# colonelwatch/ESP32-fluid-simulation

Measured on AMD Instinct MI355X. Metric: cell-iters/sec (SOR sweep), higher is better.
Workload: dtype f32

## Files before the change

esp32-fluid-simulation_amd/__init__.py:

```python
from . import _capi as capi
from ._capi import LIB_PATH, SflError, build_library
from .solver import (BatchSolver, HostPath, Solver, comm_unique_id, device_count, device_info, plan_poisson,
                     member_params, member_stops, slab_rows, sor_pass_plan, stdout_to_stderr, FLOW_STATS_DTYPE,
                     FLOW_STATS_STRIP_COLS, FLOW_STATS_CHUNK_ROWS, FIELD_DISTANCE_DTYPE, DIST_THREADS, DIST_ITEM_LOADS,
                     DIST_VELOCITY_LANE_CELLS, DIST_PRESSURE_LANE_CELLS, DIST_DYE_LANE_CELLS, ENV_BLOCK_WORDS,
                     ENV_GROUP_MEMBERS, View, PALETTE_GREY, PALETTE_HEAT, PALETTE_BLUE_WHITE_RED)

__all__ = ["capi", "LIB_PATH", "SflError", "build_library", "BatchSolver", "HostPath", "Solver",
           "comm_unique_id", "device_count", "device_info", "member_params", "member_stops", "plan_poisson", "slab_rows",
           "sor_pass_plan", "stdout_to_stderr", "FLOW_STATS_DTYPE", "FLOW_STATS_STRIP_COLS", "FLOW_STATS_CHUNK_ROWS",
           "FIELD_DISTANCE_DTYPE", "DIST_THREADS", "DIST_ITEM_LOADS", "DIST_VELOCITY_LANE_CELLS", "DIST_PRESSURE_LANE_CELLS",
           "DIST_DYE_LANE_CELLS", "ENV_BLOCK_WORDS", "ENV_GROUP_MEMBERS", "View", "PALETTE_GREY", "PALETTE_HEAT",
           "PALETTE_BLUE_WHITE_RED"]
```

esp32-fluid-simulation_amd/_capi.py:

```python
from __future__ import annotations

import ctypes as C
import os
import subprocess

_PKG = os.path.dirname(os.path.abspath(__file__))
LIB_PATH = os.path.join(_PKG, "lib", "libsfl_hip.so")

OK, ERR_INVALID, ERR_HIP, ERR_RCCL, ERR_NOMEM, ERR_STATE, ERR_HALO = 0, -1, -2, -3, -4, -5, -6
FIELD_VELOCITY, FIELD_COLOR, FIELD_DIVERGENCE, FIELD_PRESSURE = 0, 1, 2, 3
OPT_SOR_KERNEL, OPT_SOR_FUSE, OPT_ADVECT_HALO, OPT_SOR_ROWS, OPT_TRANSPORT = 0, 1, 2, 3, 4
OPT_SOR_LANE_CELLS = 5
OPT_SOR_HALO = 6
OPT_FUSE_PROJECTION = 7
OPT_ADVECT_KERNEL = 9
OPT_FUSE_DIVERGENCE = 10
OPT_SMALL_GRID = 11
OPT_EMULATE_WIRE_US = 12
OPT_STEP_SEAMS = 14
OPT_LAST_EARLY_ROWS = 17
OPT_HALO_TIMEOUT_MS = 18
OPT_EXCHANGE_SCHEDULE = 19
SCHEDULE_AUTO, SCHEDULE_IN_LINE, SCHEDULE_BY_EVENT, SCHEDULE_IN_TIME = 0, 1, 2, 3
OPT_MEASURED_WIRE_US = 20
# ... 127 lines not shown
    "sfl_distance": (_i, [_ctx, _ctx, _i, C.POINTER(FieldDistance)]),
    "sfl_step": (_i, [_ctx, _f, _f, _i, _f]),
    "sfl_step_n": (_i, [_ctx, _i, _f, _f, _i, _f]),
    "sfl_queue_forces": (_i, [_ctx, _pi, _pf, _i]),
    "sfl_queue_drags": (_i, [_ctx, C.c_void_p, _i]),
    "sfl_queue_forces_at": (_i, [_ctx, _i, _pi, _pf, _i]),
    "sfl_queue_drags_at": (_i, [_ctx, _i, C.c_void_p, _i]),
    "sfl_forces_pending": (_i, [_ctx, _pi, _pi]),
    "sfl_forget_forces": (_i, [_ctx]),
    "sfl_setup_sketch_fields": (_i, [_ctx]),
    "sfl_render_rgb565": (_i, [_ctx, _i, _i, C.POINTER(C.c_uint16), _sz]),
    "sfl_synchronize": (_i, [_ctx]),
    "sfl_timer_start": (_i, [_ctx]),
    "sfl_timer_stop": (_i, [_ctx, _pf]),
    "sfl_last_solve_info": (_i, [_ctx, _pi, _pi, _pi]),
    "sfl_batch_create": (_i, [C.POINTER(_ctx), _i, _i, _i, _i]),
    "sfl_batch_create_large": (_i, [C.POINTER(_ctx), _i, _i, _i, _i]),
    "sfl_batch_is_large": (_i, [_ctx, _pi]),
    "sfl_batch_destroy": (_i, [_ctx]),
    "sfl_batch_shape": (_i, [_ctx, _pi, _pi, _pi]),
    "sfl_batch_upload": (_i, [_ctx, _i, _i, _i, C.c_void_p, _sz]),
    "sfl_batch_download": (_i, [_ctx, _i, _i, _i, C.c_void_p, _sz]),
    "sfl_batch_field_device_ptr": (_i, [_ctx, _i, C.POINTER(C.c_void_p)]),
    "sfl_batch_queue_forces": (_i, [_ctx, _pi, _pi, _pf, _i]),
    "sfl_batch_queue_forces_at": (_i, [_ctx, _i, _pi, _pi, _pf, _i]),
    "sfl_batch_forces_pending": (_i, [_ctx, _pi, _pi]),
    "sfl_batch_forget_forces": (_i, [_ctx]),
    "sfl_batch_step_n": (_i, [_ctx, _i, _f, _f, _i, _f]),
    "sfl_batch_poisson_solve": (_i, [_ctx, _f, _i, _f]),
    "sfl_batch_step_n_each": (_i, [_ctx, _i, C.POINTER(MemberParams)]),
# ... 54 lines not shown
```

esp32-fluid-simulation_amd/csrc/sor_executor.cpp:

```cpp
#include "transport.h"

namespace sfl {
namespace host {

static bool quarter_omega_is_exact(float omega) { return (-0.25f * omega) * -4.0f == omega; }

sfl::SorParams sor_params(const sfl_context *c, float dx, float omega)
{
    sfl::SorParams prm;
    prm.dx = dx;
    prm.omega = omega;
    prm.one_minus_omega = 1.0f - omega;
    prm.neg_quarter_omega = -0.25f * omega;
    prm.fold = c->opt.sor_fold && quarter_omega_is_exact(omega) ? 1 : 0;
    return prm;
}

int effective_fuse(const sfl_context *c)
{
    int f = c->opt.sor_fuse;
    if (f == 0) {
        const int64_t cells = (int64_t)min_owned_rows(c) * c->dim_x;
        f = cells >= 12000000 ? 16 : cells >= 3000000 ? 10 : 8;
    }
// ... 389 lines not shown
        const sfl_plan_step &last = progs[k].back();
        if (last.kind != SFL_STEP_SOR) tail = 0;
        if (c->rank > 0) tail = std::min(tail, c->g0 - last.g_begin);
        if (c->rank < c->nranks - 1) tail = std::min(tail, last.g_end - c->g1);
    }
    for (sfl_context *c : peers) c->p_ghost_valid = tail > 0 ? tail : 0;
    if (timed_solve >= 0) {
        SFL_TRY(use_device(ctx));
        HIP_TRY(hipEventRecord(tuner.ev[2 * timed_solve + 1], ctx->stream));
    }
    return SFL_OK;
}

}
}
```

esp32-fluid-simulation_amd/csrc/sor_fused.hip:

```cpp
#include <cstdio>
#include <cstdlib>

#include "kernels.h"
#include "sor_stream_core.h"

#ifndef SFL_DX_PART
#define SFL_DX_PART (-1)
#endif

namespace sfl {
namespace {

constexpr int kWavesPerBlock = 4;
#ifndef SFL_NT_STORE_CELLS
#define SFL_NT_STORE_CELLS (24u << 20)
#endif
constexpr size_t kNtStoreCells = SFL_NT_STORE_CELLS;
constexpr int kFlipTiles = 1;
constexpr int kThreads = 64 * kWavesPerBlock;

#include "sor_lane.h"

#ifndef SFL_MIN_WAVES_DEEP
#define SFL_MIN_WAVES_DEEP 3
#endif
// ... 11 lines not shown
        B bk;
        bk.rs_p = __builtin_amdgcn_make_buffer_rsrc(const_cast<float *>(ZERO_IN ? d : p_in), 0, records, 0x00020000);
        bk.rs_d = __builtin_amdgcn_make_buffer_rsrc(const_cast<float *>(d), 0, records, 0x00020000);
        bk.rs_out = __builtin_amdgcn_make_buffer_rsrc(p_out, 0, records, 0x00020000);
        bk.dim_x = g.dim_x;
        bk.gdim_y = g.gdim_y;
        bk.grow0 = g.grow0;
        bk.row_lo = max(g.grow0, 0);
        bk.row_hi = min(g.grow0 + g.lrows, g.gdim_y);
        bk.row_sign = 1;
        bk.prio_on = sender ? 2 : t.rotate;
        bk.start_turns();
        bk.setup(ring_base, lane, x0, t.halo_cols);
        return bk;
    };
    if (sor::tile_touches_boundary(t, rect, g.gdim_y)) {
        B bk = backend();
        sor::Consts<B> c{bk.splat(prm.dx), bk.splat(prm.omega), bk.splat(prm.one_minus_omega), bk.splat(prm.neg_quarter_omega)};
        const auto eca = bk.edge_cell(lane, x0, 0);
        const auto ecb = bk.edge_cell(lane, x0, 1);
        sor::stream_tile<B, NS, true, DX1, ZERO_IN>(bk, c, eca, ecb, r0, r1);
        return 1;
    }
    if (sor::tile_may_flip(t, rect)) {
        B bk = backend();
        bk.row_sign = -1;
        sor::Consts<B> c{bk.splat(prm.dx), bk.splat(prm.omega), bk.splat(prm.one_minus_omega), bk.splat(prm.neg_quarter_omega)};
        const sor::EdgeCell<B> none{};
        sor::stream_tile<B, NS, false, DX1, ZERO_IN, true>(bk, c, none, none, 1 - r1, 1 - r0);
        return 2;
    }
    B bk = backend();
    sor::Consts<B> c{bk.splat(prm.dx), bk.splat(prm.omega), bk.splat(prm.one_minus_omega), bk.splat(prm.neg_quarter_omega)};
    const sor::EdgeCell<B> none{};
    sor::stream_tile<B, NS, false, DX1, ZERO_IN>(bk, c, none, none, r0, r1);
    return 0;
}

__device__ __forceinline__ int tile_of_wave(int wave, int free_blocks)
{
    int block = blockIdx.x;
    if (block < free_blocks) {
        const int per = free_blocks >> 3, rem = free_blocks & 7;
        const int xcd = block & 7, idx = block >> 3;
        block = xcd * per + min(xcd, rem) + idx;
    }
    return block * kWavesPerBlock + wave;
}

template <class B, int NS, bool DX1, bool ZERO_IN>
__global__ void __launch_bounds__(kThreads) __attribute__((amdgpu_waves_per_eu(min_waves_per_simd(NS))))
// ... 65 lines not shown
inline int device_simds()
{
    static int cached = 0;
    if (cached) return cached;
    int dev = 0, cus = 0;
    if (hipGetDevice(&dev) != hipSuccess ||
        hipDeviceGetAttribute(&cus, hipDeviceAttributeMultiprocessorCount, dev) != hipSuccess || cus < 1) {
        (void)hipGetLastError();
        return 1024;
    }
    cached = cus * 4;
    return cached;
}

template <class B>
int auto_rows_per_chunk(const Slab &g, int g_begin, int g_end, int ns, int waves, int simds, int edge_cost16)
{
    const int rows = g_end - g_begin;
    int best_rows = rows;
    double best_cost = 1e300;
    const int max_chunks = (rows + 7) / 8;
    for (int chunks = 1; chunks <= max_chunks; ++chunks) {
        const int rpc = (rows + chunks - 1) / chunks;
        const sor::Tiling t = sor::make_tiling(ns, B::kTileCols, B::kColAlign, g.dim_x, g.gdim_y, g_begin,
                                               g_end, rpc, edge_cost16, kFlipTiles);
        const long tiles = t.n_tiles;
        const double per_simd = (double)tiles / simds;
        const long serial = (tiles + simds - 1) / simds;
        const long rounds = (tiles + waves - 1) / waves;
        const double penalty = per_simd >= 2.8 ? 1.0 : per_simd >= 1.9 ? 1.08 : 1.45;
        double cost = (double)(serial > rounds ? serial : rounds) * (rpc + ns + 2) * penalty;
        if (cost < best_cost - 1e-9) {
            best_cost = cost;
            best_rows = rpc;
        }
        if (tiles > 12L * simds) break;
    }
    return best_rows;
}

struct LaunchPlan {
    sor::Tiling t1, t2;
    HaloWait hw;
    int blocks;
    int rot_c, rot_e, free_blocks;
    int senders;
};

template <class B, int NS, bool DX1, bool ZERO_IN>
LaunchPlan plan_launch(Slab g, SorRows rows, int rows_per_chunk, int sweep, const HaloWait *wait)
{
    LaunchPlan pl{};
    auto tiling = [&](int g_begin, int g_end) {
        if (g_end <= g_begin) {
            sor::Tiling none{};
            none.n_tiles = 0;
            return none;
        }
        const int resident = resident_waves<B, NS, DX1, ZERO_IN>();
        auto with_edge_cost = [&](int cost16) {
            int rpc = rows_per_chunk > g_end - g_begin ? g_end - g_begin : rows_per_chunk;
            if (rpc <= 0) rpc = auto_rows_per_chunk<B>(g, g_begin, g_end, NS, resident, device_simds(), cost16);
            return sor::make_tiling(NS, B::kTileCols, B::kColAlign, g.dim_x, g.gdim_y, g_begin, g_end, rpc, cost16,
                                    kFlipTiles ? 1 + (sweep & 1) : 0);
        };
        const sor::Tiling t = with_edge_cost(sor::kEdgeRowCost16);
        return t.n_tiles > resident ? with_edge_cost(sor::kEdgeRowCostQueued16) : t;
    };
    sor::Tiling &t1 = pl.t1, &t2 = pl.t2;
    t1 = tiling(rows.g_begin, rows.g_end);
    t2 = tiling(rows.g2_begin, rows.g2_end);
    const int tiles = t1.n_tiles + t2.n_tiles;
    if (tiles == 0) return pl;
    t1.rotate = t2.rotate = SFL_PRIO_FORCE >= 0 ? SFL_PRIO_FORCE
// ... 8 lines not shown
        const int reach = NS + sor::ring_rows(NS) + line_rows;
        auto free_range = [&](int strip, int n_chunks, int *c0, int *count) {
            *c0 = *count = 0;
            for (int c = 0; c < n_chunks; ++c) {
                const sor::TileRect r = sor::tile_rect(t1, sor::tile_index(t1, strip, c));
                if (r.r0 - reach < hw.own_lo || r.r1 + reach > hw.own_hi) continue;
                if (*count == 0) *c0 = c;
                ++*count;
            }
        };
        int fc = 0, fe = 0;
        if (t1.n_inner > 0) free_range(1, t1.n_chunks, &pl.rot_c, &fc);
        free_range(0, t1.n_chunks_edge, &pl.rot_e, &fe);
        pl.free_blocks = fc * t1.n_inner / kWavesPerBlock;
    }
    if (hw.done)
        for (const sor::Tiling *t : {&t1, &t2})
            for (int k = 0; k < t->n_tiles; ++k) {
                const sor::TileRect r = sor::tile_rect(*t, k);
                pl.senders += r.r0 < hw.send_lo_end || r.r1 > hw.send_hi_begin;
            }
    return pl;
}

template <class B, int NS, bool DX1, bool ZERO_IN>
hipError_t launch_variant(hipStream_t s, float *p_out, const float *p_in, const float *d, Slab g,
                          SorRows rows, SorParams prm, int rows_per_chunk, int sweep, const HaloWait *wait, int *senders)
{
    const LaunchPlan pl = plan_launch<B, NS, DX1, ZERO_IN>(g, rows, rows_per_chunk, sweep, wait);
    if (pl.blocks == 0) return hipSuccess;
    if (senders) *senders = pl.senders;
    sor_fused_kernel<B, NS, DX1, ZERO_IN><<<pl.blocks, kThreads, 0, s>>>(p_out, p_in, d, g, pl.t1, pl.t2, prm, pl.hw, pl.rot_c, pl.rot_e,
                                                                        pl.free_blocks);
    return hipGetLastError();
}

template <class B, int NS, bool ZERO_IN>
hipError_t launch_dx(hipStream_t s, float *p_out, const float *p_in, const float *d, Slab g,
                     SorRows rows, SorParams prm, int rows_per_chunk, int sweep, const HaloWait *wait, int *senders)
{
#if SFL_DX_PART != 1
    if (prm.dx == 1.0f)
        return launch_variant<B, NS, true, ZERO_IN>(s, p_out, p_in, d, g, rows, prm, rows_per_chunk, sweep, wait, senders);
#endif
#if SFL_DX_PART != 0
    if (prm.dx != 1.0f)
// ... 115 lines not shown
```

esp32-fluid-simulation_amd/csrc/sor_lane.h:

```cpp
#pragma once

typedef float v2f __attribute__((ext_vector_type(2)));
typedef int v2i __attribute__((ext_vector_type(2)));

#ifndef SFL_PRIO_LEVELS
#define SFL_PRIO_LEVELS 4
#endif
#ifndef SFL_PRIO_FORCE
#define SFL_PRIO_FORCE (-1)
#endif
#ifndef SFL_PRIO_ROWS
#define SFL_PRIO_ROWS 2
#endif
#ifndef SFL_SCALAR_PRODUCTS
#define SFL_SCALAR_PRODUCTS 1
#endif

__device__ __forceinline__ float lane_below(float x)
{
    return __builtin_bit_cast(float, __builtin_amdgcn_update_dpp(0, __builtin_bit_cast(int, x), 0x138, 0xf, 0xf, false));
}
__device__ __forceinline__ float lane_above(float x)
{
    return __builtin_bit_cast(float, __builtin_amdgcn_update_dpp(0, __builtin_bit_cast(int, x), 0x130, 0xf, 0xf, false));
// ... 53 lines not shown
    }
    __device__ __forceinline__ int row_bytes(int t) const { return (row_sign * t - grow0) * dim_x * 4; }
    __device__ __forceinline__ int load_row_bytes(int t) const
    {
        return (min(max(row_sign * t, row_lo), row_hi - 1) - grow0) * dim_x * 4;
    }
};

template <int NS, bool VEC, bool ZERO_IN, int ST = 0, bool FOLD = false>
struct Lane2 : WaveCommon {
    using V = float;
    using M = bool;
    static constexpr bool kFoldQuarter = FOLD;
    static constexpr int kTileCols = 128, kColAlign = 2, kCells = 2, kPrefetch = 3, kTurnRows = SFL_PRIO_ROWS;
    static constexpr int kStoreAux = VEC ? ST : 0;
    static constexpr int kRingFloats = sor::ring_rows(NS) * 2 * 64;

    float *ring;
    int off_a, off_b;
    int off_out;
    bool a_out, b_out;

    __device__ __forceinline__ void setup(float *ring_base, int lane, int x0, int halo)
    {
        ring = ring_base + lane;
        const int xa = x0 + 2 * lane;
        if (VEC) {
            off_a = 4 * min(max(xa, 0), dim_x - 2);
            off_b = off_a + 4;
        } else {
            off_a = 4 * min(max(xa, 0), dim_x - 1);
            off_b = 4 * min(max(xa + 1, 0), dim_x - 1);
        }
        off_out = 4 * xa;
        const int out_lo = x0 + halo, out_hi = x0 + kTileCols - halo;
        a_out = xa >= 0 && xa < dim_x && xa >= out_lo && xa < out_hi;
        b_out = xa + 1 >= 0 && xa + 1 < dim_x && xa + 1 >= out_lo && xa + 1 < out_hi;
    }
    __device__ __forceinline__ sor::EdgeCell<Lane2> edge_cell(int lane, int x0, int which) const
    {
        const int x = x0 + 2 * lane + which;
        sor::EdgeCell<Lane2> ec;
        const int nh = (x > 0 ? 1 : 0) + (x < dim_x - 1 ? 1 : 0);
        const float k2 = (float)(-1.0 / 2.0), k3 = (float)(-1.0 / 3.0), k4 = -0.25f;
        ec.in = x >= 0 && x < dim_x;
        ec.k_full = (nh == 2) ? k4 : (nh == 1) ? k3 : k2;
        ec.k_part = (nh == 2) ? k3 : k2;
        ec.z_full = (nh == 2) ? -0.0f : 0.0f;
        return ec;
    }

    __device__ __forceinline__ V splat(float x) const { return x; }
    __device__ __forceinline__ V select(M m, V a, V b) const { return m ? a : b; }
    __device__ __forceinline__ M mask_and(M m, bool row) const { return m && row; }
    __device__ __forceinline__ V from_lower_lane(V x) const { return lane_below(x); }
    __device__ __forceinline__ V from_upper_lane(V x) const { return lane_above(x); }
    __device__ __forceinline__ V scalar_only(V x) const
    {
#if SFL_SCALAR_PRODUCTS
        asm("" : "+v"(x));
#endif
        return x;
    }
    __device__ __forceinline__ V detach(V x) const
// ... 55 lines not shown
```

esp32-fluid-simulation_amd/csrc/sor_stream_core.h:

```cpp
#pragma once
#include <type_traits>
#include <utility>

#ifndef SFL_EDGE_PROLOGUE_MAX_NS
#define SFL_EDGE_PROLOGUE_MAX_NS 12
#endif

#if defined(__HIPCC__)
#define SFL_HD __host__ __device__ __forceinline__
#else
#define SFL_HD inline
#endif

namespace sfl {
namespace sor {


constexpr int wrapn(int x, int n) { return ((x % n) + n) % n; }
constexpr bool is_even(int x) { return ((x % 2) + 2) % 2 == 0; }
constexpr int ring_rows(int ns) { return ((ns + 1 + 5) / 6) * 6; }

template <class B>
struct EdgeCell {
    typename B::M in;
// ... 42 lines not shown
    using V = typename B::V;
    const V rhs = d;
    if (!EDGE) {
        const V sum = ((w + e) + s) + n;
        if (!B::kFoldQuarter) return c.one_minus_omega * own + scalar_only(bk, c.omega * (bk.splat(-0.25f) * (rhs - sum)));
        return c.one_minus_omega * own + scalar_only(bk, c.neg_quarter_omega * (rhs - sum));
    }
    const V z = rf.full ? ec.z_full : bk.splat(0.0f);
    const V k = rf.full ? ec.k_full : ec.k_part;
    const V sum = (((z + w) + e) + s) + n;
    const V gs = k * (rhs - sum);
    const V out = c.one_minus_omega * own + c.omega * gs;
    return bk.select(bk.mask_and(ec.in, rf.in_dom), out, bk.splat(-0.0f));
}

constexpr int kRhsAhead = 1;
constexpr int kSteadyTrip = 2;
constexpr bool pass_runs(int trip, int ring, int u, int s)
{
    return trip >= kSteadyTrip || trip * ring + u >= 2 * s;
}
constexpr bool edge_prologue(int ns) { return ns <= SFL_EDGE_PROLOGUE_MAX_NS; }
constexpr int prologue_trips(int ns) { return (2 * ns + ring_rows(ns) - 1) / ring_rows(ns); }
constexpr bool steady_rows_are_output(int ns) { return prologue_trips(ns) * ring_rows(ns) >= 2 * ns + 1; }

template <class B, int NS, bool EDGE, bool DX1, bool ZERO_IN, int TRIP, bool GUARD_STORE, bool FLIP, int U>
SFL_HD void iterate(B &bk, Pipe<B, NS> &pp, const Consts<B> &c, const EdgeCell<B> &eca,
                    const EdgeCell<B> &ecb, int y, int out_begin, int out_end)
{
    using V = typename B::V;
    constexpr int RING = ring_rows(NS);
    constexpr int kPrefetch = B::kPrefetch;
    constexpr int Q = U % kPrefetch;

    if (U % B::kTurnRows == 0) bk.next_turn();

    {
        V a = bk.detach(pp.pa[Q]), b = bk.detach(pp.pb[Q]);
        const V fa = DX1 ? pp.da[Q] : c.dx * pp.da[Q], fb = DX1 ? pp.db[Q] : c.dx * pp.db[Q];
        bk.ring_store(U, 0, is_even(U) ? fa : fb);
        bk.ring_store(U, 1, is_even(U) ? fb : fa);
        bk.load_row(y + kPrefetch, pp.pa[Q], pp.pb[Q], pp.da[Q], pp.db[Q]);
        if (ZERO_IN) a = b = bk.splat(0.0f);
        if (EDGE) {
            const RowFacts rf = bk.row_facts(y);
            a = bk.select(bk.mask_and(eca.in, rf.in_dom), a, bk.splat(-0.0f));
            b = bk.select(bk.mask_and(ecb.in, rf.in_dom), b, bk.splat(-0.0f));
        }
        constexpr bool ev = is_even(U);
        pp.E[U] = ev ? a : b;
        pp.O[U] = ev ? b : a;
    }

    constexpr int kAhead = kRhsAhead;
    V d_e[NS / 2 + 1], d_o[NS / 2 + 1];
#pragma unroll
    for (int m = 1; m <= kAhead && m <= NS / 2; ++m) {
        d_e[m] = bk.ring_load(wrapn(U - (2 * m - 1), RING), 0);
        d_o[m] = bk.ring_load(wrapn(U - 2 * m, RING), 1);
    }
#pragma unroll
    for (int m = 1; m <= NS / 2; ++m) {
        if (m + kAhead <= NS / 2) {
            d_e[m + kAhead] = bk.ring_load(wrapn(U - (2 * (m + kAhead) - 1), RING), 0);
            d_o[m + kAhead] = bk.ring_load(wrapn(U - 2 * (m + kAhead), RING), 1);
            bk.pin();
        }
        if (pass_runs(TRIP, RING, U, 2 * m - 1)) {
            const int lag = 2 * m - 1;
            const int r = y - lag;
            const int rel = U - lag;
            const int i0 = wrapn(rel, RING), im = wrapn(rel - 1, RING), ip = wrapn(rel + 1, RING);
            const bool ev = is_even(rel);
            const V own = pp.E[i0];
            const V oc = pp.O[i0];
            const V w = ev ? bk.from_lower_lane(oc) : oc;
            const V e = ev ? oc : bk.from_upper_lane(oc);
            const V d = d_e[m];
            const RowFacts rf = bk.row_facts(r);
            pp.E[i0] = relax<B, EDGE>(bk, c, own, w, e, pp.O[FLIP ? ip : im], pp.O[FLIP ? im : ip], d,
                                           ev ? eca : ecb, rf);
        }
        if (pass_runs(TRIP, RING, U, 2 * m)) {
            const int lag = 2 * m;
            const int r = y - lag;
            const int rel = U - lag;
            const int i0 = wrapn(rel, RING), im = wrapn(rel - 1, RING), ip = wrapn(rel + 1, RING);
            const bool ev = is_even(rel);
            const V own = pp.O[i0];
            const V oc = pp.E[i0];
            const V w = ev ? oc : bk.from_lower_lane(oc);
            const V e = ev ? bk.from_upper_lane(oc) : oc;
            const V d = d_o[m];
            const RowFacts rf = bk.row_facts(r);
            const V res = relax<B, EDGE>(bk, c, own, w, e, pp.E[FLIP ? ip : im], pp.E[FLIP ? im : ip], d,
                                              ev ? ecb : eca, rf);
            if (m < NS / 2) {
                pp.O[i0] = res;
            } else if (!GUARD_STORE || (r >= out_begin && r < out_end)) {
                if (ev)
                    bk.store_row(r, oc, res);
                else
                    bk.store_row(r, res, oc);
            }
        }
    }
}

template <class B, int NS, bool EDGE, bool DX1, bool ZERO_IN, int TRIP, bool PARTIAL, bool FLIP, int... Us>
SFL_HD void run_unrolled(B &bk, Pipe<B, NS> &pp, const Consts<B> &c, const EdgeCell<B> &eca,
                         const EdgeCell<B> &ecb, int y, int out_begin, int out_end,
                         std::integer_sequence<int, Us...>)
{
    const int y_stop = out_end + NS;
    constexpr bool guard = PARTIAL || TRIP < kSteadyTrip || !steady_rows_are_output(NS) ||
                           (EDGE && !edge_prologue(NS));
    (void)(((!PARTIAL || y + Us < y_stop) &&
            (iterate<B, NS, EDGE, DX1, ZERO_IN, TRIP, guard, FLIP, Us>(bk, pp, c, eca, ecb, y + Us, out_begin,
                                                                       out_end),
             true)) && ...);
}

template <class B, int NS, bool EDGE, bool DX1, bool ZERO_IN, bool FLIP = false>
SFL_HD void stream_tile(B &bk, const Consts<B> &c, const EdgeCell<B> &eca,
                        const EdgeCell<B> &ecb, int out_begin, int out_end)
{
    static_assert(NS >= 2 && NS % 2 == 0, "fuse an even number of colour passes");
    constexpr int RING = ring_rows(NS);
    constexpr int kPrefetch = B::kPrefetch;
    static_assert(RING % 6 == 0 && 6 % kPrefetch == 0 && RING >= NS + 1, "ring geometry");
    Pipe<B, NS> pp;
    bk.poison(pp);

// ... 8 lines not shown
    if ((!EDGE || edge_prologue(NS)) && y + RING <= y_stop) {
        run_unrolled<B, NS, EDGE, DX1, ZERO_IN, 0, false, FLIP>(bk, pp, c, eca, ecb, y, out_begin, out_end, us);
        y += RING;
        if (prologue_trips(NS) >= 2 && y + RING <= y_stop) {
                run_unrolled<B, NS, EDGE, DX1, ZERO_IN, 1, false, FLIP>(bk, pp, c, eca, ecb, y, out_begin, out_end, us);
            y += RING;
        }
    }
    static_assert(prologue_trips(NS) <= kSteadyTrip, "prologue trips");
    for (; y + RING <= y_stop; y += RING)
        run_unrolled<B, NS, EDGE, DX1, ZERO_IN, kSteadyTrip, false, FLIP>(bk, pp, c, eca, ecb, y, out_begin,
                                                                    out_end, us);
    if (y < y_stop)
        run_unrolled<B, NS, EDGE, DX1, ZERO_IN, kSteadyTrip, true, FLIP>(bk, pp, c, eca, ecb, y, out_begin,
                                                                   out_end, us);
}

struct Tiling {
    int ns;
    int dim_x;
    int g_begin, g_end;
    int rows_per_chunk;
    int rows_edge;
    int rows_first;
    int rows_last;
    int n_strips;
    int n_inner;
    int n_chunks;
    int n_chunks_edge;
    int n_tiles;
    int tile_cols, halo_cols;
    int rotate;
    int flip;
};

struct TileRect {
    int strip;
    int r0, r1;
    int flip;
};

SFL_HD int strip_step(const Tiling &t) { return t.tile_cols - 2 * t.halo_cols; }

SFL_HD int strip_x0(const Tiling &t, int strip) { return strip * strip_step(t) - t.halo_cols; }

#ifndef SFL_EDGE_ROW_COST16
#define SFL_EDGE_ROW_COST16 10
#endif
// ... 2 lines not shown
constexpr int kMinEdgeRows = 8;
SFL_HD int balanced_edge_rows(int rows_per_chunk, int ns, int sixteenths)
{
    const int warm = edge_prologue(ns) ? ns : 2 * ns;
    const int r = (rows_per_chunk + ns) * sixteenths / 16 - warm;
    if (r >= kMinEdgeRows) return r;
    return (kMinEdgeRows + warm) * 16 * 5 <= (rows_per_chunk + ns) * sixteenths * 6 ? kMinEdgeRows : 0;
}

SFL_HD Tiling make_tiling(int ns, int tile_cols, int col_align, int dim_x, int gdim_y, int g_begin,
                          int g_end, int rows_per_chunk, int balance16, int flip = 0)
{
    Tiling t;
    t.rotate = 0;
    t.flip = flip;
    const int rows = g_end - g_begin;
    t.ns = ns;
    t.dim_x = dim_x;
    t.g_begin = g_begin;
    t.g_end = g_end;
    t.rows_per_chunk = rows_per_chunk;
    t.tile_cols = tile_cols;
    t.halo_cols = (ns + col_align - 1) / col_align * col_align;
    t.n_strips = (dim_x + strip_step(t) - 1) / strip_step(t);

    int n_right = 0;
    while (n_right < t.n_strips && strip_x0(t, t.n_strips - 1 - n_right) + tile_cols >= dim_x) ++n_right;
    t.n_inner = t.n_strips - 1 - n_right;
    if (t.n_inner < 0) t.n_inner = 0;

// ... 73 lines not shown
    return t.n_inner * t.n_chunks + (strip == 0 ? 0 : strip - t.n_inner) * t.n_chunks_edge + chunk;
}

SFL_HD bool tile_may_flip(const Tiling &t, const TileRect &r)
{
    return r.flip && r.r0 - t.ns - ring_rows(t.ns) > 0;
}

SFL_HD bool tile_touches_boundary(const Tiling &t, const TileRect &r, int gdim_y)
{
    const int x0 = strip_x0(t, r.strip);
    return x0 <= 0 || x0 + t.tile_cols >= t.dim_x || r.r0 - t.ns - 1 <= 0 ||
           r.r1 + t.ns + ring_rows(t.ns) >= gdim_y;
}

}
}
```

esp32-fluid-simulation_amd/solver.py:

```python
from __future__ import annotations

import ctypes as C

import numpy as np

from . import _capi as capi

_FIELD_SPEC = {
    capi.FIELD_VELOCITY: (np.float32, 2),
    capi.FIELD_COLOR: (np.uint32, 3),
    capi.FIELD_DIVERGENCE: (np.float32, 1),
    capi.FIELD_PRESSURE: (np.float32, 1),
}


MEMBER_PARAMS_DTYPE = np.dtype([("dt", "<f4"), ("dx", "<f4"), ("omega", "<f4"), ("iters", "<i4")])


def member_params(batch: int, dt, dx=1.0, iters=10, omega=1.96) -> np.ndarray:
    out = np.empty(batch, MEMBER_PARAMS_DTYPE)
    for name, value in (("dt", dt), ("dx", dx), ("omega", omega), ("iters", iters)):
        a = np.asarray(value)
        if a.ndim > 1 or (a.ndim == 1 and len(a) != batch):
            raise ValueError(f"{name}: a scalar or a sequence of {batch} values (one per member), got shape {a.shape}")
# ... 54 lines not shown
    return name.value.decode(), cus.value, mem.value


def slab_rows(dim_y: int, nranks: int, rank: int):
    b, e = C.c_int(), C.c_int()
    capi.check(capi.lib().sfl_slab_rows(dim_y, nranks, rank, C.byref(b), C.byref(e)))
    return b.value, e.value


def sor_pass_plan(iters: int, fuse: int):
    n = C.c_int()
    capi.check(capi.lib().sfl_sor_pass_plan(iters, fuse, C.byref(n), None, 0))
    arr = (C.c_int * max(n.value, 1))()
    capi.check(capi.lib().sfl_sor_pass_plan(iters, fuse, C.byref(n), arr, n.value))
    return list(arr[: n.value])


def plan_poisson(dim_y: int, nranks: int, rank: int, iters: int, fuse: int = 8, kernel: int = 2,
                 halo: int = 0, tail: int = 0):
    n = C.c_int()
    capi.check(capi.lib().sfl_plan_poisson_tail(dim_y, nranks, rank, iters, fuse, kernel, halo, tail, None, 0,
                                                C.byref(n)))
    steps = (capi.PlanStep * max(n.value, 1))()
    capi.check(capi.lib().sfl_plan_poisson_tail(dim_y, nranks, rank, iters, fuse, kernel, halo, tail, steps,
                                                n.value, C.byref(n)))
    return [steps[k] for k in range(n.value)]


class stdout_to_stderr:

# ... 662 lines not shown
```

include/sfl.h:

```cpp
#ifndef SFL_H
#define SFL_H

#include <stddef.h>
#include <stdint.h>

#ifdef __cplusplus
extern "C" {
#endif

#define SFL_API __attribute__((visibility("default")))

#define SFL_ABI_VERSION 1

#define SFL_OK 0
#define SFL_ERR_INVALID (-1)
#define SFL_ERR_HIP (-2)
#define SFL_ERR_RCCL (-3)
#define SFL_ERR_NOMEM (-4)
#define SFL_ERR_STATE (-5)
#define SFL_ERR_HALO (-6)

#define SFL_FIELD_VELOCITY 0
#define SFL_FIELD_COLOR 1
#define SFL_FIELD_DIVERGENCE 2
// ... 137 lines not shown
SFL_API int sfl_queue_drags(sfl_context *ctx, const sfl_drag *msgs, int n);
SFL_API int sfl_queue_forces_at(sfl_context *ctx, int step, const int *cells_ij, const float *vel_xy, int n);
SFL_API int sfl_queue_drags_at(sfl_context *ctx, int step, const sfl_drag *msgs, int n);
SFL_API int sfl_forces_pending(sfl_context *ctx, int *records, int *last_step);
SFL_API int sfl_forget_forces(sfl_context *ctx);

SFL_API int sfl_setup_sketch_fields(sfl_context *ctx);

SFL_API int sfl_render_rgb565(sfl_context *ctx, int scaling, int byteswap, uint16_t *host_image,
                              size_t bytes);

SFL_API int sfl_synchronize(sfl_context *ctx);
SFL_API int sfl_timer_start(sfl_context *ctx);
SFL_API int sfl_timer_stop(sfl_context *ctx, float *elapsed_ms);
SFL_API int sfl_last_solve_info(sfl_context *ctx, int *launches, int *exchanges, int *fuse);


SFL_API int sfl_batch_create(sfl_batch **out, int device, int dim_x, int dim_y, int batch);
#define SFL_BATCH_LARGE_MAX_CELLS 20224
SFL_API int sfl_batch_create_large(sfl_batch **out, int device, int dim_x, int dim_y, int batch);
SFL_API int sfl_batch_is_large(sfl_batch *b, int *large);
SFL_API int sfl_batch_destroy(sfl_batch *b);
SFL_API int sfl_batch_shape(sfl_batch *b, int *dim_x, int *dim_y, int *batch);
SFL_API int sfl_batch_upload(sfl_batch *b, int field, int first, int count, const void *host, size_t bytes);
SFL_API int sfl_batch_download(sfl_batch *b, int field, int first, int count, void *host, size_t bytes);
SFL_API int sfl_batch_field_device_ptr(sfl_batch *b, int field, void **dev_ptr);
SFL_API int sfl_batch_queue_forces(sfl_batch *b, const int *members, const int *cells_ij, const float *vel_xy, int n);
SFL_API int sfl_batch_queue_forces_at(sfl_batch *b, int step, const int *members, const int *cells_ij,
                                      const float *vel_xy, int n);
SFL_API int sfl_batch_forces_pending(sfl_batch *b, int *records, int *last_step);
// ... 91 lines not shown
```

Measured before the change: 3064 billion.

## Add wall-aligned SOR tiling with specialized boundary-row paths

Adds a new tiling mode for the fused SOR kernel. Strips are anchored to the left and right domain walls and own variable column ranges, so no column edge masking is needed. Tiles at the top and bottom walls get compile-time wall variants that fold the Neumann partial coefficient (-1/2 at walls) into a specialized relax, instead of going through the generic masked edge path. This should cut how many tiles take the slow edge path, at the cost of more template instantiations, code size and register pressure. It is on by default for vectorised non-fold backends, can be disabled with an environment variable, and adds a host-side tile-path counter exposed through a new C/Python API.

```diff
diff --git a/esp32-fluid-simulation_amd/__init__.py b/esp32-fluid-simulation_amd/__init__.py
--- a/esp32-fluid-simulation_amd/__init__.py
+++ b/esp32-fluid-simulation_amd/__init__.py
@@ -1,14 +1,14 @@
 from . import _capi as capi
 from ._capi import LIB_PATH, SflError, build_library
 from .solver import (BatchSolver, HostPath, Solver, comm_unique_id, device_count, device_info, plan_poisson,
-                     member_params, member_stops, slab_rows, sor_pass_plan, stdout_to_stderr, FLOW_STATS_DTYPE,
+                     member_params, member_stops, slab_rows, sor_last_tile_paths, sor_pass_plan, stdout_to_stderr, FLOW_STATS_DTYPE,
                      FLOW_STATS_STRIP_COLS, FLOW_STATS_CHUNK_ROWS, FIELD_DISTANCE_DTYPE, DIST_THREADS, DIST_ITEM_LOADS,
                      DIST_VELOCITY_LANE_CELLS, DIST_PRESSURE_LANE_CELLS, DIST_DYE_LANE_CELLS, ENV_BLOCK_WORDS,
                      ENV_GROUP_MEMBERS, View, PALETTE_GREY, PALETTE_HEAT, PALETTE_BLUE_WHITE_RED)
 
 __all__ = ["capi", "LIB_PATH", "SflError", "build_library", "BatchSolver", "HostPath", "Solver",
            "comm_unique_id", "device_count", "device_info", "member_params", "member_stops", "plan_poisson", "slab_rows",
-           "sor_pass_plan", "stdout_to_stderr", "FLOW_STATS_DTYPE", "FLOW_STATS_STRIP_COLS", "FLOW_STATS_CHUNK_ROWS",
+           "sor_last_tile_paths", "sor_pass_plan", "stdout_to_stderr", "FLOW_STATS_DTYPE", "FLOW_STATS_STRIP_COLS", "FLOW_STATS_CHUNK_ROWS",
            "FIELD_DISTANCE_DTYPE", "DIST_THREADS", "DIST_ITEM_LOADS", "DIST_VELOCITY_LANE_CELLS", "DIST_PRESSURE_LANE_CELLS",
            "DIST_DYE_LANE_CELLS", "ENV_BLOCK_WORDS", "ENV_GROUP_MEMBERS", "View", "PALETTE_GREY", "PALETTE_HEAT",
            "PALETTE_BLUE_WHITE_RED"]
diff --git a/esp32-fluid-simulation_amd/_capi.py b/esp32-fluid-simulation_amd/_capi.py
--- a/esp32-fluid-simulation_amd/_capi.py
+++ b/esp32-fluid-simulation_amd/_capi.py
@@ -165,6 +165,7 @@
     "sfl_timer_start": (_i, [_ctx]),
     "sfl_timer_stop": (_i, [_ctx, _pf]),
     "sfl_last_solve_info": (_i, [_ctx, _pi, _pi, _pi]),
+    "sfl_sor_last_tile_paths": (_i, [_pi]),
     "sfl_batch_create": (_i, [C.POINTER(_ctx), _i, _i, _i, _i]),
     "sfl_batch_create_large": (_i, [C.POINTER(_ctx), _i, _i, _i, _i]),
     "sfl_batch_is_large": (_i, [_ctx, _pi]),
diff --git a/esp32-fluid-simulation_amd/csrc/sor_executor.cpp b/esp32-fluid-simulation_amd/csrc/sor_executor.cpp
--- a/esp32-fluid-simulation_amd/csrc/sor_executor.cpp
+++ b/esp32-fluid-simulation_amd/csrc/sor_executor.cpp
@@ -1,6 +1,9 @@
+#include <atomic>
+
 #include "transport.h"
 
 namespace sfl {
+std::atomic<int> g_sor_last_tile_paths[5];
 namespace host {
 
 static bool quarter_omega_is_exact(float omega) { return (-0.25f * omega) * -4.0f == omega; }
@@ -427,3 +430,10 @@
 
 }
 }
+
+extern "C" int sfl_sor_last_tile_paths(int counts[5])
+{
+    if (!counts) return SFL_ERR_INVALID;
+    for (int k = 0; k < 5; ++k) counts[k] = sfl::g_sor_last_tile_paths[k].load(std::memory_order_relaxed);
+    return SFL_OK;
+}
diff --git a/esp32-fluid-simulation_amd/csrc/sor_fused.hip b/esp32-fluid-simulation_amd/csrc/sor_fused.hip
--- a/esp32-fluid-simulation_amd/csrc/sor_fused.hip
+++ b/esp32-fluid-simulation_amd/csrc/sor_fused.hip
@@ -1,6 +1,8 @@
 #include <cstdio>
 #include <cstdlib>
 
+#include <atomic>
+
 #include "kernels.h"
 #include "sor_stream_core.h"
 
@@ -9,6 +11,7 @@
 #endif
 
 namespace sfl {
+extern std::atomic<int> g_sor_last_tile_paths[5];
 namespace {
 
 constexpr int kWavesPerBlock = 4;
@@ -50,6 +53,45 @@
         bk.setup(ring_base, lane, x0, t.halo_cols);
         return bk;
     };
+    if constexpr (B::kWallTiles) {
+        int xw = x0, lo = x0 + t.halo_cols, hi = x0 + B::kTileCols - t.halo_cols, path;
+        if (t.wall) {
+            xw = sor::strip_x0_wall(t, rect.strip);
+            sor::strip_owned(t, rect.strip, &lo, &hi);
+            path = sor::wall_tile_path(t, rect, g.gdim_y);
+        } else {
+            path = sor::tile_touches_boundary(t, rect, g.gdim_y) ? sor::kPathEdge : sor::tile_may_flip(t, rect) ? sor::kPathDown : sor::kPathUp;
+        }
+        auto run = [&](auto flip, auto wall, int out_begin, int out_end) {
+            B bk = backend();
+            bk.setup_owned(ring_base, lane, xw, lo, hi);
+            if (flip) bk.row_sign = -1;
+            sor::Consts<B> c{bk.splat(prm.dx), bk.splat(prm.omega), bk.splat(prm.one_minus_omega), bk.splat(prm.neg_quarter_omega)};
+            const auto eca = bk.edge_cell(lane, xw, 0);
+            const auto ecb = bk.edge_cell(lane, xw, 1);
+            sor::stream_tile_wall<B, NS, DX1, ZERO_IN, decltype(flip)::value, decltype(wall)::value>(bk, c, eca, ecb, out_begin, out_end);
+        };
+        using std::integral_constant;
+        if (path == sor::kPathEdge) {
+            B bk = backend();
+            bk.setup_owned(ring_base, lane, xw, lo, hi);
+            sor::Consts<B> c{bk.splat(prm.dx), bk.splat(prm.omega), bk.splat(prm.one_minus_omega), bk.splat(prm.neg_quarter_omega)};
+            const auto eca = bk.edge_cell(lane, xw, 0);
+            const auto ecb = bk.edge_cell(lane, xw, 1);
+            sor::stream_tile<B, NS, true, DX1, ZERO_IN>(bk, c, eca, ecb, r0, r1);
+        } else if (path == sor::kPathDown) {
+            run(integral_constant<bool, true>{}, integral_constant<int, 0>{}, 1 - r1, 1 - r0);
+        } else if (path == sor::kPathUp) {
+            run(integral_constant<bool, false>{}, integral_constant<int, 0>{}, r0, r1);
+        } else if (path == sor::kPathBottomWall) {
+            run(integral_constant<bool, false>{}, integral_constant<int, 1>{}, r0, r1);
+        } else if ((1 - r1) & 1) {
+            run(integral_constant<bool, true>{}, integral_constant<int, 2>{}, 1 - r1, 1 - r0);
+        } else {
+            run(integral_constant<bool, true>{}, integral_constant<int, 1>{}, 1 - r1, 1 - r0);
+        }
+        return path;
+    } else {
     if (sor::tile_touches_boundary(t, rect, g.gdim_y)) {
         B bk = backend();
         sor::Consts<B> c{bk.splat(prm.dx), bk.splat(prm.omega), bk.splat(prm.one_minus_omega), bk.splat(prm.neg_quarter_omega)};
@@ -71,6 +113,7 @@
     const sor::EdgeCell<B> none{};
     sor::stream_tile<B, NS, false, DX1, ZERO_IN>(bk, c, none, none, r0, r1);
     return 0;
+    }
 }
 
 __device__ __forceinline__ int tile_of_wave(int wave, int free_blocks)
@@ -166,7 +209,7 @@
 }
 
 template <class B>
-int auto_rows_per_chunk(const Slab &g, int g_begin, int g_end, int ns, int waves, int simds, int edge_cost16)
+int auto_rows_per_chunk(const Slab &g, int g_begin, int g_end, int ns, int waves, int simds, int edge_cost16, bool wall = false)
 {
     const int rows = g_end - g_begin;
     int best_rows = rows;
@@ -174,8 +217,9 @@
     const int max_chunks = (rows + 7) / 8;
     for (int chunks = 1; chunks <= max_chunks; ++chunks) {
         const int rpc = (rows + chunks - 1) / chunks;
-        const sor::Tiling t = sor::make_tiling(ns, B::kTileCols, B::kColAlign, g.dim_x, g.gdim_y, g_begin,
-                                               g_end, rpc, edge_cost16, kFlipTiles);
+        const sor::Tiling t = wall ? sor::make_tiling_wall(ns, B::kTileCols, B::kColAlign, g.dim_x, g.gdim_y, g_begin, g_end, rpc, kFlipTiles)
+                                   : sor::make_tiling(ns, B::kTileCols, B::kColAlign, g.dim_x, g.gdim_y, g_begin,
+                                                      g_end, rpc, edge_cost16, kFlipTiles);
         const long tiles = t.n_tiles;
         const double per_simd = (double)tiles / simds;
         const long serial = (tiles + simds - 1) / simds;
@@ -191,13 +235,41 @@
     return best_rows;
 }
 
+template <class B>
+bool wall_tiles_wanted(int dim_x)
+{
+    if (!B::kWallTiles || !sor::wall_tiling_fits(B::kTileCols, dim_x)) return false;
+    const char *e = getenv("SFL_SOR_WALL_TILES");
+    return !(e && e[0] == '0');
+}
+
 struct LaunchPlan {
     sor::Tiling t1, t2;
     HaloWait hw;
     int blocks;
     int rot_c, rot_e, free_blocks;
     int senders;
+    int paths[sor::kTilePaths];
 };
+
+template <class B>
+void count_tile_paths(LaunchPlan &pl, int gdim_y)
+{
+    for (const sor::Tiling *t : {&pl.t1, &pl.t2}) {
+        if (t->n_tiles == 0) continue;
+        auto walk = [&](int strip, int n_chunks, int strips) {
+            for (int c = 0; c < n_chunks; ++c) {
+                const sor::TileRect r = sor::tile_rect(*t, sor::tile_index(*t, strip, c));
+                const int path = B::kWallTiles && t->wall ? sor::wall_tile_path(*t, r, gdim_y)
+                                 : sor::tile_touches_boundary(*t, r, gdim_y) ? sor::kPathEdge
+                                 : sor::tile_may_flip(*t, r) ? sor::kPathDown : sor::kPathUp;
+                pl.paths[path] += strips;
+            }
+        };
+        if (t->n_inner > 0) walk(1, t->n_chunks, t->n_inner);
+        walk(0, t->n_chunks_edge, t->n_strips - t->n_inner);
+    }
+}
 
 template <class B, int NS, bool DX1, bool ZERO_IN>
 LaunchPlan plan_launch(Slab g, SorRows rows, int rows_per_chunk, int sweep, const HaloWait *wait)
@@ -210,6 +282,12 @@
             return none;
         }
         const int resident = resident_waves<B, NS, DX1, ZERO_IN>();
+        if (wall_tiles_wanted<B>(g.dim_x)) {
+            int rpc = rows_per_chunk > g_end - g_begin ? g_end - g_begin : rows_per_chunk;
+            if (rpc <= 0) rpc = auto_rows_per_chunk<B>(g, g_begin, g_end, NS, resident, device_simds(), 0, true);
+            return sor::make_tiling_wall(NS, B::kTileCols, B::kColAlign, g.dim_x, g.gdim_y, g_begin, g_end, rpc,
+                                         kFlipTiles ? 1 + (sweep & 1) : 0);
+        }
         auto with_edge_cost = [&](int cost16) {
             int rpc = rows_per_chunk > g_end - g_begin ? g_end - g_begin : rows_per_chunk;
             if (rpc <= 0) rpc = auto_rows_per_chunk<B>(g, g_begin, g_end, NS, resident, device_simds(), cost16);
@@ -248,6 +326,7 @@
         free_range(0, t1.n_chunks_edge, &pl.rot_e, &fe);
         pl.free_blocks = fc * t1.n_inner / kWavesPerBlock;
     }
+    count_tile_paths<B>(pl, g.gdim_y);
     if (hw.done)
         for (const sor::Tiling *t : {&t1, &t2})
             for (int k = 0; k < t->n_tiles; ++k) {
@@ -264,6 +343,7 @@
     const LaunchPlan pl = plan_launch<B, NS, DX1, ZERO_IN>(g, rows, rows_per_chunk, sweep, wait);
     if (pl.blocks == 0) return hipSuccess;
     if (senders) *senders = pl.senders;
+    for (int k = 0; k < sor::kTilePaths; ++k) g_sor_last_tile_paths[k].store(pl.paths[k], std::memory_order_relaxed);
     sor_fused_kernel<B, NS, DX1, ZERO_IN><<<pl.blocks, kThreads, 0, s>>>(p_out, p_in, d, g, pl.t1, pl.t2, prm, pl.hw, pl.rot_c, pl.rot_e,
                                                                         pl.free_blocks);
     return hipGetLastError();
diff --git a/esp32-fluid-simulation_amd/csrc/sor_lane.h b/esp32-fluid-simulation_amd/csrc/sor_lane.h
--- a/esp32-fluid-simulation_amd/csrc/sor_lane.h
+++ b/esp32-fluid-simulation_amd/csrc/sor_lane.h
@@ -91,6 +91,7 @@
     static constexpr bool kFoldQuarter = FOLD;
     static constexpr int kTileCols = 128, kColAlign = 2, kCells = 2, kPrefetch = 3, kTurnRows = SFL_PRIO_ROWS;
     static constexpr int kStoreAux = VEC ? ST : 0;
+    static constexpr bool kWallTiles = VEC && !FOLD;
     static constexpr int kRingFloats = sor::ring_rows(NS) * 2 * 64;
 
     float *ring;
@@ -99,6 +100,10 @@
     bool a_out, b_out;
 
     __device__ __forceinline__ void setup(float *ring_base, int lane, int x0, int halo)
+    {
+        setup_owned(ring_base, lane, x0, x0 + halo, x0 + kTileCols - halo);
+    }
+    __device__ __forceinline__ void setup_owned(float *ring_base, int lane, int x0, int out_lo, int out_hi)
     {
         ring = ring_base + lane;
         const int xa = x0 + 2 * lane;
@@ -110,7 +115,6 @@
             off_b = 4 * min(max(xa + 1, 0), dim_x - 1);
         }
         off_out = 4 * xa;
-        const int out_lo = x0 + halo, out_hi = x0 + kTileCols - halo;
         a_out = xa >= 0 && xa < dim_x && xa >= out_lo && xa < out_hi;
         b_out = xa + 1 >= 0 && xa + 1 < dim_x && xa + 1 >= out_lo && xa + 1 < out_hi;
     }
@@ -125,6 +129,12 @@
         ec.k_part = (nh == 2) ? k3 : k2;
         ec.z_full = (nh == 2) ? -0.0f : 0.0f;
         return ec;
+    }
+
+    __device__ __forceinline__ V part_k(int which) const
+    {
+        const int x = (off_out >> 2) + which;
+        return (x > 0 && x < dim_x - 1) ? (float)(-1.0 / 3.0) : (float)(-1.0 / 2.0);
     }
 
     __device__ __forceinline__ V splat(float x) const { return x; }
diff --git a/esp32-fluid-simulation_amd/csrc/sor_stream_core.h b/esp32-fluid-simulation_amd/csrc/sor_stream_core.h
--- a/esp32-fluid-simulation_amd/csrc/sor_stream_core.h
+++ b/esp32-fluid-simulation_amd/csrc/sor_stream_core.h
@@ -80,6 +80,19 @@
     return bk.select(bk.mask_and(ec.in, rf.in_dom), out, bk.splat(-0.0f));
 }
 
+template <class B>
+SFL_HD typename B::V relax_wall(const B &bk, const Consts<B> &c, typename B::V own, typename B::V w, typename B::V e,
+                                typename B::V s, typename B::V n, typename B::V d, const EdgeCell<B> &ec, bool wall_row)
+{
+    using V = typename B::V;
+    if (!wall_row) {
+        const V sum = ((w + e) + s) + n;
+        return c.one_minus_omega * own + scalar_only(bk, c.omega * (ec.k_full * (d - sum)));
+    }
+    const V sum = (((bk.splat(0.0f) + w) + e) + s) + n;
+    return c.one_minus_omega * own + scalar_only(bk, c.omega * (ec.k_part * (d - sum)));
+}
+
 constexpr int kRhsAhead = 1;
 constexpr int kSteadyTrip = 2;
 constexpr bool pass_runs(int trip, int ring, int u, int s)
@@ -90,7 +103,10 @@
 constexpr int prologue_trips(int ns) { return (2 * ns + ring_rows(ns) - 1) / ring_rows(ns); }
 constexpr bool steady_rows_are_output(int ns) { return prologue_trips(ns) * ring_rows(ns) >= 2 * ns + 1; }
 
-template <class B, int NS, bool EDGE, bool DX1, bool ZERO_IN, int TRIP, bool GUARD_STORE, bool FLIP, int U>
+constexpr int kWallNone = 0, kWallK = 1, kWallTrip0 = 2, kWallTrip1 = 3;
+constexpr bool wall_pass_runs(int wall, int u, int s) { return u - s >= wall - kWallTrip0; }
+
+template <class B, int NS, bool EDGE, bool DX1, bool ZERO_IN, int TRIP, bool GUARD_STORE, bool FLIP, int WALL, int U>
 SFL_HD void iterate(B &bk, Pipe<B, NS> &pp, const Consts<B> &c, const EdgeCell<B> &eca,
                     const EdgeCell<B> &ecb, int y, int out_begin, int out_end)
 {
@@ -108,6 +124,7 @@
         bk.ring_store(U, 1, is_even(U) ? fb : fa);
         bk.load_row(y + kPrefetch, pp.pa[Q], pp.pb[Q], pp.da[Q], pp.db[Q]);
         if (ZERO_IN) a = b = bk.splat(0.0f);
+        if (WALL >= kWallTrip0 && U < WALL - kWallTrip0) a = b = bk.splat(-0.0f);
         if (EDGE) {
             const RowFacts rf = bk.row_facts(y);
             a = bk.select(bk.mask_and(eca.in, rf.in_dom), a, bk.splat(-0.0f));
@@ -132,7 +149,7 @@
             d_o[m + kAhead] = bk.ring_load(wrapn(U - 2 * (m + kAhead), RING), 1);
             bk.pin();
         }
-        if (pass_runs(TRIP, RING, U, 2 * m - 1)) {
+        if (WALL >= kWallTrip0 ? wall_pass_runs(WALL, U, 2 * m - 1) : pass_runs(TRIP, RING, U, 2 * m - 1)) {
             const int lag = 2 * m - 1;
             const int r = y - lag;
             const int rel = U - lag;
@@ -144,10 +161,14 @@
             const V e = ev ? oc : bk.from_upper_lane(oc);
             const V d = d_e[m];
             const RowFacts rf = bk.row_facts(r);
-            pp.E[i0] = relax<B, EDGE>(bk, c, own, w, e, pp.O[FLIP ? ip : im], pp.O[FLIP ? im : ip], d,
+            if (WALL != kWallNone)
+                pp.E[i0] = relax_wall<B>(bk, c, own, w, e, pp.O[FLIP ? ip : im], pp.O[FLIP ? im : ip], d, ev ? eca : ecb,
+                                         WALL >= kWallTrip0 && rel == WALL - kWallTrip0);
+            else
+                pp.E[i0] = relax<B, EDGE>(bk, c, own, w, e, pp.O[FLIP ? ip : im], pp.O[FLIP ? im : ip], d,
                                            ev ? eca : ecb, rf);
         }
-        if (pass_runs(TRIP, RING, U, 2 * m)) {
+        if (WALL >= kWallTrip0 ? wall_pass_runs(WALL, U, 2 * m) : pass_runs(TRIP, RING, U, 2 * m)) {
             const int lag = 2 * m;
             const int r = y - lag;
             const int rel = U - lag;
@@ -159,8 +180,11 @@
             const V e = ev ? bk.from_upper_lane(oc) : oc;
             const V d = d_o[m];
             const RowFacts rf = bk.row_facts(r);
-            const V res = relax<B, EDGE>(bk, c, own, w, e, pp.E[FLIP ? ip : im], pp.E[FLIP ? im : ip], d,
-                                              ev ? ecb : eca, rf);
+            const V res = WALL != kWallNone
+                              ? relax_wall<B>(bk, c, own, w, e, pp.E[FLIP ? ip : im], pp.E[FLIP ? im : ip], d, ev ? ecb : eca,
+                                              WALL >= kWallTrip0 && rel == WALL - kWallTrip0)
+                              : relax<B, EDGE>(bk, c, own, w, e, pp.E[FLIP ? ip : im], pp.E[FLIP ? im : ip], d,
+                                               ev ? ecb : eca, rf);
             if (m < NS / 2) {
                 pp.O[i0] = res;
             } else if (!GUARD_STORE || (r >= out_begin && r < out_end)) {
@@ -173,7 +197,7 @@
     }
 }
 
-template <class B, int NS, bool EDGE, bool DX1, bool ZERO_IN, int TRIP, bool PARTIAL, bool FLIP, int... Us>
+template <class B, int NS, bool EDGE, bool DX1, bool ZERO_IN, int TRIP, bool PARTIAL, bool FLIP, int WALL = kWallNone, int... Us>
 SFL_HD void run_unrolled(B &bk, Pipe<B, NS> &pp, const Consts<B> &c, const EdgeCell<B> &eca,
                          const EdgeCell<B> &ecb, int y, int out_begin, int out_end,
                          std::integer_sequence<int, Us...>)
@@ -182,7 +206,7 @@
     constexpr bool guard = PARTIAL || TRIP < kSteadyTrip || !steady_rows_are_output(NS) ||
                            (EDGE && !edge_prologue(NS));
     (void)(((!PARTIAL || y + Us < y_stop) &&
-            (iterate<B, NS, EDGE, DX1, ZERO_IN, TRIP, guard, FLIP, Us>(bk, pp, c, eca, ecb, y + Us, out_begin,
+            (iterate<B, NS, EDGE, DX1, ZERO_IN, TRIP, guard, FLIP, WALL, Us>(bk, pp, c, eca, ecb, y + Us, out_begin,
                                                                        out_end),
              true)) && ...);
 }
@@ -221,6 +245,59 @@
     if (y < y_stop)
         run_unrolled<B, NS, EDGE, DX1, ZERO_IN, kSteadyTrip, true, FLIP>(bk, pp, c, eca, ecb, y, out_begin,
                                                                    out_end, us);
+}
+
+template <class B, class = void>
+struct has_part_k : std::false_type {};
+template <class B>
+struct has_part_k<B, std::void_t<decltype(&B::part_k)>> : std::true_type {};
+
+template <class B, int NS, bool DX1, bool ZERO_IN, bool FLIP, int wall>
+SFL_HD void stream_tile_wall(B &bk, const Consts<B> &c, const EdgeCell<B> &eca, const EdgeCell<B> &ecb, int out_begin,
+                             int out_end)
+{
+    static_assert(NS >= 2 && NS % 2 == 0, "fuse an even number of colour passes");
+    constexpr int RING = ring_rows(NS);
+    constexpr int kPrefetch = B::kPrefetch;
+    static_assert(RING % 6 == 0 && 6 % kPrefetch == 0 && RING >= NS + 2, "ring geometry");
+    Pipe<B, NS> pp;
+    bk.poison(pp);
+
+    int y = out_begin - NS;
+    y -= (y & 1);
+    if (wall) y = out_begin - (wall - 1);
+    const int y_stop = out_end + NS;
+
+#pragma unroll
+    for (int u = 0; u < kPrefetch; ++u) bk.load_row(y + u, pp.pa[u], pp.pb[u], pp.da[u], pp.db[u]);
+
+    constexpr auto us = std::make_integer_sequence<int, RING>{};
+    if constexpr (wall != 0) {
+        EdgeCell<B> wa = eca, wb = ecb;
+        if constexpr (has_part_k<B>::value) {
+            wa.k_part = bk.part_k(0);
+            wb.k_part = bk.part_k(1);
+        }
+        if constexpr (wall == 1) {
+            pp.E[RING - 1] = pp.O[RING - 1] = bk.splat(-0.0f);
+            run_unrolled<B, NS, false, DX1, ZERO_IN, 0, false, FLIP, kWallTrip0>(bk, pp, c, wa, wb, y, out_begin, out_end, us);
+        } else {
+            run_unrolled<B, NS, false, DX1, ZERO_IN, 0, false, FLIP, kWallTrip1>(bk, pp, c, wa, wb, y, out_begin, out_end, us);
+        }
+        y += RING;
+        
+    } else if (y + RING <= y_stop) {
+        run_unrolled<B, NS, false, DX1, ZERO_IN, 0, false, FLIP, kWallK>(bk, pp, c, eca, ecb, y, out_begin, out_end, us);
+        y += RING;
+        if (prologue_trips(NS) >= 2 && y + RING <= y_stop) {
+            run_unrolled<B, NS, false, DX1, ZERO_IN, 1, false, FLIP, kWallK>(bk, pp, c, eca, ecb, y, out_begin, out_end, us);
+            y += RING;
+        }
+    }
+    for (; y + RING <= y_stop; y += RING)
+        run_unrolled<B, NS, false, DX1, ZERO_IN, kSteadyTrip, false, FLIP, kWallK>(bk, pp, c, eca, ecb, y, out_begin, out_end, us);
+    if (y < y_stop)
+        run_unrolled<B, NS, false, DX1, ZERO_IN, kSteadyTrip, true, FLIP, kWallK>(bk, pp, c, eca, ecb, y, out_begin, out_end, us);
 }
 
 struct Tiling {
@@ -239,6 +316,7 @@
     int tile_cols, halo_cols;
     int rotate;
     int flip;
+    int wall;
 };
 
 struct TileRect {
@@ -271,6 +349,7 @@
     Tiling t;
     t.rotate = 0;
     t.flip = flip;
+    t.wall = 0;
     const int rows = g_end - g_begin;
     t.ns = ns;
     t.dim_x = dim_x;
@@ -374,5 +453,58 @@
            r.r1 + t.ns + ring_rows(t.ns) >= gdim_y;
 }
 
-}
-}
+SFL_HD bool wall_tiling_fits(int tile_cols, int dim_x) { return dim_x >= tile_cols && (dim_x & 1) == 0; }
+
+SFL_HD Tiling make_tiling_wall(int ns, int tile_cols, int col_align, int dim_x, int gdim_y, int g_begin, int g_end,
+                               int rows_per_chunk, int flip = 0)
+{
+    Tiling t;
+    (void)gdim_y;
+    t.rotate = 0;
+    t.flip = flip;
+    t.wall = 1;
+    t.ns = ns;
+    t.dim_x = dim_x;
+    t.g_begin = g_begin;
+    t.g_end = g_end;
+    t.rows_per_chunk = t.rows_edge = rows_per_chunk;
+    t.rows_first = t.rows_last = 0;
+    t.tile_cols = tile_cols;
+    t.halo_cols = (ns + col_align - 1) / col_align * col_align;
+    t.n_strips = 1 + (dim_x - tile_cols + strip_step(t) - 1) / strip_step(t);
+    t.n_inner = t.n_strips > 2 ? t.n_strips - 2 : 0;
+    t.n_chunks = t.n_chunks_edge = (g_end - g_begin + rows_per_chunk - 1) / rows_per_chunk;
+    t.n_tiles = t.n_strips * t.n_chunks;
+    return t;
+}
+
+SFL_HD int strip_x0_wall(const Tiling &t, int strip)
+{
+    return strip == t.n_strips - 1 ? t.dim_x - t.tile_cols : strip * strip_step(t);
+}
+
+SFL_HD void strip_owned(const Tiling &t, int strip, int *lo, int *hi)
+{
+    *lo = strip == 0 ? 0 : strip * strip_step(t) + t.halo_cols;
+    *hi = strip == t.n_strips - 1 ? t.dim_x : (strip + 1) * strip_step(t) + t.halo_cols;
+}
+
+enum TilePath { kPathUp = 0, kPathEdge = 1, kPathDown = 2, kPathBottomWall = 3, kPathTopWall = 4, kTilePaths = 5 };
+SFL_HD int wall_tile_path(const Tiling &t, const TileRect &r, int gdim_y)
+{
+    const int ring = ring_rows(t.ns);
+    const bool bottom = r.r0 <= 0, top = r.r1 >= gdim_y;
+    const bool room_below = r.r0 - t.ns - ring > 0;
+    const bool room_above = r.r1 + t.ns + ring < gdim_y;
+    const bool full_trip = r.r1 - r.r0 + t.ns >= ring;
+    if (bottom || top) {
+        if (bottom && top) return kPathEdge;
+        if (bottom) return full_trip && room_above ? kPathBottomWall : kPathEdge;
+        return full_trip && room_below ? kPathTopWall : kPathEdge;
+    }
+    if (r.r0 - t.ns - 1 <= 0 || !room_above) return kPathEdge;
+    return r.flip && room_below ? kPathDown : kPathUp;
+}
+
+}
+}
diff --git a/esp32-fluid-simulation_amd/solver.py b/esp32-fluid-simulation_amd/solver.py
--- a/esp32-fluid-simulation_amd/solver.py
+++ b/esp32-fluid-simulation_amd/solver.py
@@ -92,6 +92,12 @@
     arr = (C.c_int * max(n.value, 1))()
     capi.check(capi.lib().sfl_sor_pass_plan(iters, fuse, C.byref(n), arr, n.value))
     return list(arr[: n.value])
+
+
+def sor_last_tile_paths():
+    arr = (C.c_int * 5)()
+    capi.check(capi.lib().sfl_sor_last_tile_paths(arr))
+    return dict(zip(("up", "edge", "down", "bottom_wall", "top_wall"), arr))
 
 
 def plan_poisson(dim_y: int, nranks: int, rank: int, iters: int, fuse: int = 8, kernel: int = 2,
diff --git a/include/sfl.h b/include/sfl.h
--- a/include/sfl.h
+++ b/include/sfl.h
@@ -175,6 +175,7 @@
 SFL_API int sfl_timer_start(sfl_context *ctx);
 SFL_API int sfl_timer_stop(sfl_context *ctx, float *elapsed_ms);
 SFL_API int sfl_last_solve_info(sfl_context *ctx, int *launches, int *exchanges, int *fuse);
+SFL_API int sfl_sor_last_tile_paths(int counts[5]);
 
 
 SFL_API int sfl_batch_create(sfl_batch **out, int device, int dim_x, int dim_y, int batch);
```

New measurement: 3024 billion. 1.3% lower.
